# yugabyte/yugabyte-db

Measured on AMD Instinct MI355X. Metric: scanned_rows_per_s, higher is better.
Workload: dtype int64; 1 GPU; 1 tablet, 100M rows, 4KB SST blocks, three_shared_parts, packed-row V2, 3 int64 predicates + SUM(int64); rows=100000000, tablets=1, block_size=4096

## Files before the change

### yugabyte-db_amd/csrc/fast_sim_main.cc

```cpp
#include <cstdio>
#include <cstdlib>
#include <cstring>
#include <vector>

#include "../../include/yb_gpu_scan.h"

extern "C" int ybg_sim_scan(const ybg_scan_spec_t*, const uint8_t*,
                            const uint64_t*, uint64_t, ybg_scan_result_t*);
extern "C" int ybg_sim_scan_fast(const ybg_scan_spec_t*, const uint8_t*,
                                 const uint64_t*, uint64_t,
                                 ybg_scan_result_t*, uint64_t*);

namespace {

constexpr uint64_t kSlack = 48;
constexpr uint64_t kMvccBase = 1600000000000000ull;

ybg_schema_t make_schema(int ncols) {
  ybg_schema_t s;
  memset(&s, 0, sizeof(s));
  s.has_hash = 1;
  s.num_hash_cols = 1;
  s.key_types[0] = YBG_KT_INT64;
  s.num_value_cols = ncols;
  for (int i = 0; i < ncols; ++i) s.value_cols[i] = {10 + i, YBG_T_INT64, 1};
  return s;
}

struct Query {
  int num_preds;
  ybg_pred_t preds[3];
  ybg_agg_t aggs[2];
  uint64_t read, local;
};

bool same(const ybg_scan_result_t& a, const ybg_scan_result_t& b) {
  bool ok = a.rows_scanned == b.rows_scanned &&
            a.rows_matched == b.rows_matched &&
            a.entries_seen == b.entries_seen &&
            a.restart_ht_len == b.restart_ht_len &&
            !memcmp(a.restart_ht, b.restart_ht, a.restart_ht_len);
  for (int g = 0; g < 2 && ok; ++g)
    ok = a.aggs[g].is_null == b.aggs[g].is_null &&
         (a.aggs[g].is_null || a.aggs[g].value_i64 == b.aggs[g].value_i64);
  return ok;
}

int check(const char* what, const ybg_schema_t& schema, const uint8_t* data,
          const uint64_t* offsets, uint64_t n_blocks, uint64_t total,
          const Query& q) {
  uint8_t* exact = (uint8_t*)malloc(total + kSlack);
  memcpy(exact, data, total);
  memset(exact + total, 0, kSlack);
  ybg_scan_spec_t spec;
  memset(&spec, 0, sizeof(spec));
  spec.schema = schema;
  spec.kv_format = YBG_ENC_THREE_SHARED_PARTS;
  ybg_read_time_init(&spec.read_time, q.read << 12, q.local << 12,
                     q.local << 12);
  spec.num_preds = q.num_preds;
  for (int i = 0; i < q.num_preds; ++i) spec.preds[i] = q.preds[i];
  spec.num_aggs = 2;
  spec.aggs[0] = q.aggs[0];
  spec.aggs[1] = q.aggs[1];
  int bad = 0;
  uint64_t nf_max = 0;
  for (const char* ivb : {"1", "2", "4"}) {
    setenv("YBG_IVB", ivb, 1);
    ybg_scan_result_t want;
    spec.expect_versions = 0;
    bad |= ybg_sim_scan(&spec, exact, offsets, n_blocks, &want);
    for (const char* plan : {"1", "0"}) {
      setenv("YBG_PLAN", plan, 1);
      for (int fuse = 0; fuse < 2; ++fuse) {
        spec.expect_versions = fuse;
        ybg_scan_result_t got;
        uint64_t nf = 0;
        int rc = ybg_sim_scan_fast(&spec, exact, offsets, n_blocks, &got, &nf);
        if (rc || !same(got, want)) {
          printf("  %s ivb=%s plan=%s fuse=%d: rc=%d MISMATCH\n", what, ivb,
                 plan, fuse, rc);
          bad = 1;
        }
        if (nf > nf_max) nf_max = nf;
      }
    }
    if (!strcmp(ivb, "1"))
      printf("%s: blocks=%llu bytes=%llu scanned=%llu matched=%llu "
             "fallbacks<=%llu %s\n",
             what, (unsigned long long)n_blocks, (unsigned long long)total,
             (unsigned long long)want.rows_scanned,
             (unsigned long long)want.rows_matched,
             (unsigned long long)nf_max, bad ? "MISMATCH" : "ok");
  }
  free(exact);
  return bad;
}

int check_generated(const char* tag, int ncols, uint64_t rows, int versions,
                    const Query& q) {
  ybg_schema_t schema = make_schema(ncols);
  ybg_gen_params_t p;
  memset(&p, 0, sizeof(p));
  p.rows = rows;
  p.seed = 42;
  p.packed_version = 2;
  p.kv_format = YBG_ENC_THREE_SHARED_PARTS;
  p.block_size = 4096;
  p.restart_interval = 16;
  p.versions = versions;
  p.ht_base_micros = kMvccBase;
  p.ht_step_micros = versions > 1 ? 1000000 : 1000;
  p.nthreads = 1;
  uint8_t* data;
  uint64_t* offsets;
  uint64_t n_blocks, total, n_entries;
  if (ybg_generate(&schema, &p, &data, &offsets, &n_blocks, &total,
                   &n_entries))
    return 1;
  char what[64];
  snprintf(what, sizeof(what), "%s rows=%llu", tag, (unsigned long long)rows);
  int bad = check(what, schema, data, offsets, n_blocks, total, q);
  ybg_free(data);
  ybg_free(offsets);
  return bad;
}

int check_built(const char* tag, int kind, uint64_t rows, const Query& q) {
  const int ncols = (kind == 1 || kind >= 4) ? 4 : 1;
  ybg_schema_t schema = make_schema(ncols);
  ybg_builder_t* b = ybg_builder_create(&schema, YBG_ENC_THREE_SHARED_PARTS,
                                        4096, kind >= 2 ? 1 : 16);
  uint64_t seq = 1ull << 50;
  int rc = 0;
  for (uint64_t r = 0; r < rows && !rc; ++r) {
    ybg_key_t k;
    memset(&k, 0, sizeof(k));
    k.hash = (uint16_t)(r / 64);
    k.datums[0] = r;
    ybg_rowvals_t v;
    memset(&v, 0, sizeof(v));
    uint64_t ht = 2000;
    if (kind == 0) {
      v.datums[0] = r * 11 + 1;
      if (r % 7 == 3) {
        rc = ybg_builder_add_row_tombstone(b, &k, 3000ull << 12, 0, seq++);
        continue;
      }
      if (r % 5 == 0)
        rc = ybg_builder_add_row_tombstone(b, &k, 3000ull << 12, 0, seq++);
    } else if (kind == 1) {
      for (int c = 0; c < 4; ++c) v.datums[c] = r * 3 + c;
      if (r % 37 == 20)
        rc = ybg_builder_add_column_update(b, &k, 2, 3000ull << 12, 0, seq++,
                                           r + 5, nullptr, 0, 0);
    } else if (kind >= 4) {
      for (int c = 0; c < 4; ++c) v.datums[c] = r * 8 + c;
      ht = 1000;
      if (kind == 5 && r + 1 == rows) {
        rc = ybg_builder_add_row_tombstone(b, &k, ht << 12, 0, seq++);
        continue;
      }
    } else {
      v.datums[0] = kind == 2 ? (uint64_t)INT64_MAX - r * 3 : r;
      ht = (kind == 3 && r == 137) ? 3000 : 1000;
    }
    if (!rc)
      rc = ybg_builder_add_packed_row(b, &k, ht << 12, 0, seq++, 2, &v);
  }
  const uint8_t* data;
  const uint64_t* offsets;
  uint64_t n_blocks, total, n_entries;
  if (rc || ybg_builder_finish(b, &data, &offsets, &n_blocks, &total,
                               &n_entries))
    return 1;
  char what[64];
  snprintf(what, sizeof(what), "%s rows=%llu", tag, (unsigned long long)rows);
  int bad = check(what, schema, data, offsets, n_blocks, total, q);
  ybg_builder_destroy(b);
  return bad;
}

}

int main() {
  const uint64_t kRead = 1700000000000000ull;
  Query headline = {3,
                    {{0, 0, YBG_PRED_GT, 1ull << 39, nullptr, 0},
                     {0, 1, YBG_PRED_LT, 3ull << 38, nullptr, 0},
                     {0, 2, YBG_PRED_GE, 1ull << 36, nullptr, 0}},
                    {{YBG_AGG_SUM_INT64, 3}, {YBG_AGG_COUNT_STAR, 0}},
                    kRead, kRead};
  Query one_col = {1,
                   {{0, 0, YBG_PRED_GT, 1ull << 39, nullptr, 0}},
                   {{YBG_AGG_COUNT_STAR, 0}, {YBG_AGG_SUM_INT64, 0}},
                   kRead, kRead};
  Query count_sum0 = {0, {}, {{YBG_AGG_COUNT_STAR, 0}, {YBG_AGG_SUM_INT64, 0}},
                      5000, 5000};
  Query mvcc = count_sum0, below = count_sum0, restart = count_sum0;
  mvcc.read = mvcc.local = kMvccBase + 2500000;
  below.read = below.local = kMvccBase - 1;
  restart.read = 2000;
  restart.local = 4000;
  Query tomb = count_sum0, upd = headline;
  tomb.num_preds = 1;
  tomb.preds[0] = {0, 0, YBG_PRED_GT, 50, nullptr, 0};
  upd.num_preds = 1;
  upd.preds[0] = {0, 0, YBG_PRED_GE, 30, nullptr, 0};
  upd.read = upd.local = 5000;

  int bad = 0;
  for (uint64_t n : {1, 2, 15, 16, 17, 31, 32, 33, 90, 91, 92, 93, 94, 182,
                     183, 184, 185, 186, 2000, 6000}) {
    bad |= check_generated("four-column", 4, n, 1, headline);
    bad |= check_generated("one-column", 1, n, 1, one_col);
  }
  bad |= check_generated("four-column", 4, 200000, 1, headline);
  for (uint64_t n : {1, 17, 33, 93, 2000}) {
    bad |= check_generated("mvcc", 4, n, 5, mvcc);
    bad |= check_generated("mvcc-below", 4, n, 5, below);
  }
  bad |= check_built("tombstones", 0, 700, tomb);
  bad |= check_built("column-update", 1, 600, upd);
  for (uint64_t n : {1, 63, 64, 65, 255, 256, 257})
    bad |= check_built("epilogue", 2, n, count_sum0);
  bad |= check_built("restart-one", 3, 200, restart);
  Query wide = headline;
  wide.num_preds = 3;
  wide.preds[0] = {0, 0, YBG_PRED_GE, 8, nullptr, 0};
  wide.preds[1] = {0, 1, YBG_PRED_LT, 8 * 90, nullptr, 0};
  wide.preds[2] = {0, 2, YBG_PRED_GE, 18, nullptr, 0};
  wide.read = wide.local = 5000;
  for (uint64_t n : {1, 2, 93, 94, 200}) {
    bad |= check_built("last-restart-sum-last-column", 4, n, wide);
    bad |= check_built("last-restart-tombstone", 5, n, wide);
  }
  printf(bad ? "FAILED\n" : "all ok\n");
  return bad;
}
```

### yugabyte-db_amd/csrc/scan_device.h

```cpp
#pragma once
#include <cstdint>
#include <cstdlib>
#include <cstring>

#include "../../include/yb_gpu_scan.h"

#ifndef YBG_DEV_QUAL
#define YBG_DEV_QUAL __device__ __forceinline__
#endif
#define DEV YBG_DEV_QUAL

#ifdef YBG_HOST_SIM
static inline double __longlong_as_double(long long v) {
  double d;
  memcpy(&d, &v, 8);
  return d;
}
static inline long long __double_as_longlong(double d) {
  long long v;
  memcpy(&v, &d, 8);
  return v;
}
static inline float __uint_as_float(unsigned v) {
  float f;
// ... 2189 lines not shown
      d = rc.emit_datums[c];
      if (((rc.emit_str >> c) & 1) && !ec->varlen) {
        d = 0;
      } else if ((rc.emit_str >> c) & 1) {
        uint32_t sl = rc.emit_lens[c];
        unsigned long long off = atomicAdd(ec->varlen_counter, sl);
        if (off + sl > ec->varlen_cap) {
          atomicAdd(ec->overflow, 1ull);
          d = 0;
        } else {
          const uint8_t* src = (const uint8_t*)(uintptr_t)d;
          for (uint32_t i = 0; i < sl; ++i) ec->varlen[off + i] = src[i];
          d = ((uint64_t)sl << 40) | off;
        }
      }
    }
    ec->datums[slot * nc + c] = d;
  }
  ec->null_masks[slot] = rc.emit_null;
  ec->hashes[slot] =
      sp.has_hash ? (uint16_t)(((uint16_t)rk[1] << 8) | rk[2]) : 0;
}


DEV void combine_datum(int op, uint64_t* val, uint64_t* cnt, uint64_t v) {
  switch (op) {
    case YBG_AGG_COUNT_STAR:
    case YBG_AGG_COUNT:
      *val += 1;
      break;
    case YBG_AGG_SUM_INT64:
      *val += v;
      break;
    case YBG_AGG_SUM_DOUBLE: {
      double cur = __longlong_as_double((long long)*val) +
                   __longlong_as_double((long long)v);
      *val = (uint64_t)__double_as_longlong(cur);
      break;
    }
    case YBG_AGG_MIN_INT64:
      if (*cnt == 0 || (int64_t)v < (int64_t)*val) *val = v;
      break;
    case YBG_AGG_MAX_INT64:
      if (*cnt == 0 || (int64_t)v > (int64_t)*val) *val = v;
      break;
    case YBG_AGG_MIN_DOUBLE: {
      double dd = __longlong_as_double((long long)v);
      if (*cnt == 0 || dd < __longlong_as_double((long long)*val))
        *val = (uint64_t)__double_as_longlong(dd);
      break;
    }
    case YBG_AGG_MAX_DOUBLE: {
      double dd = __longlong_as_double((long long)v);
      if (*cnt == 0 || dd > __longlong_as_double((long long)*val))
        *val = (uint64_t)__double_as_longlong(dd);
      break;
    }
  }
  *cnt += 1;
}

DEV bool pred_cmp_fast(const PredC& pr, uint64_t datum) {
  const int dtype = (int)(pr.opdt >> 8);
  int cmp;
  if (YBG_LIKELY(dtype != YBG_T_DOUBLE && dtype != YBG_T_FLOAT)) {
    int64_t a = (int64_t)datum, b = (int64_t)pr.datum;
    cmp = a < b ? -1 : (a > b ? 1 : 0);
  } else if (dtype == YBG_T_DOUBLE) {
    double a = __longlong_as_double((long long)datum);
    double b = __longlong_as_double((long long)pr.datum);
    cmp = a < b ? -1 : (a > b ? 1 : 0);
  } else {
    float a = __uint_as_float((uint32_t)datum);
    float b = __uint_as_float((uint32_t)pr.datum);
    cmp = a < b ? -1 : (a > b ? 1 : 0);
  }
  switch (pr.opdt & 0xff) {
    case YBG_PRED_GT: return cmp > 0;
    case YBG_PRED_GE: return cmp >= 0;
    case YBG_PRED_LT: return cmp < 0;
    case YBG_PRED_LE: return cmp <= 0;
    case YBG_PRED_EQ: return cmp == 0;
    default: return cmp != 0;
  }
}

inline bool fast_eligible(const DevSpec& d) {
  if (d.fmt != YBG_ENC_THREE_SHARED_PARTS) return false;
  if (!d.fixed_rk_len || d.need_rowkey || d.group_col >= 0) return false;
  if (!d.v2_fixed_len || d.num_value_cols <= 0) return false;
  if (d.num_value_cols > 8) return false;
  if (d.num_aggs > 2) return false;
  for (int i = 0; i < d.num_preds; ++i) {
    if (d.preds[i].is_key_col) return false;
    if (d.preds[i].op > YBG_PRED_NE) return false;
  }
  return true;
}

constexpr int kPlanMaxCols = 8;
constexpr int kPlanAggs = 2;
constexpr int kPlanGroupSlots = 4;
constexpr int kPlanShapeP1 = 16;
constexpr int kPlanShapeP1S1 = 17;
constexpr int kPlanShapeP2 = 18;
constexpr int plan_np(int nc) {
  return nc == kPlanShapeP2 ? 2 : (nc >= kPlanShapeP1 ? 1 : 0);
}
constexpr int plan_ns(int nc) {
  return nc < kPlanShapeP1 ? nc : (nc == kPlanShapeP1S1 ? 1 : 0);
}

struct FastPlan {
  int64_t lo[kPlanMaxCols], hi[kPlanMaxCols];
  uint8_t off[kPlanMaxCols];
  uint32_t n_rng;
  uint32_t agg_off[kPlanAggs];
  uint32_t agg_mask[kPlanAggs];
  uint32_t agg_one[kPlanAggs];
  uint32_t agg_on[kPlanAggs];
  uint32_t shape;
  uint32_t agg_sel[kPlanAggs][kPlanGroupSlots];
  uint32_t rkb, v2_fixed_len, track_restart;
  HtLim reg_lim;
};

inline bool build_fast_plan(const DevSpec& d, FastPlan* pl) {
  memset(pl, 0, sizeof(*pl));
  for (int k = 0; k < kPlanMaxCols; ++k) {
    pl->lo[k] = INT64_MIN;
    pl->hi[k] = INT64_MAX;
  }
  if (!fast_eligible(d) || d.num_aggs > kPlanAggs) return false;
  auto wide = [&](int c) {
    return c >= 0 && c < d.num_value_cols && d.cols[c].v2_fixed == 8;
  };
  int rng_of[YBG_MAX_COLS];
  for (int c = 0; c < YBG_MAX_COLS; ++c) rng_of[c] = -1;
  for (int i = 0; i < d.num_preds; ++i) {
    const DevPred& pr = d.preds[i];
    if (pr.op < YBG_PRED_GT || pr.op > YBG_PRED_EQ) return false;
    if (!wide(pr.col)) return false;
    const int dt = d.cols[pr.col].dtype;
    if (dt != YBG_T_INT64 && dt != YBG_T_UINT64) return false;
    if (rng_of[pr.col] < 0) {
      rng_of[pr.col] = (int)pl->n_rng;
      pl->off[pl->n_rng++] = d.v2_off[pr.col];
    }
    const int k = rng_of[pr.col];
    const int64_t c = (int64_t)pr.datum;
    int64_t lo = INT64_MIN, hi = INT64_MAX;
    bool empty = false;
    switch (pr.op) {
      case YBG_PRED_GT:
        if (c == INT64_MAX) empty = true; else lo = c + 1;
        break;
      case YBG_PRED_GE: lo = c; break;
      case YBG_PRED_LT:
        if (c == INT64_MIN) empty = true; else hi = c - 1;
        break;
      case YBG_PRED_LE: hi = c; break;
      default: lo = hi = c; break;
    }
    if (lo > pl->lo[k]) pl->lo[k] = lo;
    if (hi < pl->hi[k]) pl->hi[k] = hi;
    if (empty || pl->lo[k] > pl->hi[k]) {
      pl->lo[k] = INT64_MAX;
      pl->hi[k] = INT64_MIN;
    }
  }
  for (int g = 0; g < d.num_aggs; ++g) {
    const int op = d.aggs[g].op;
    pl->agg_on[g] = 1;
    if (op == YBG_AGG_COUNT_STAR) {
      pl->agg_one[g] = 1;
    } else if (op == YBG_AGG_COUNT) {
      if (d.aggs[g].col < 0 || d.aggs[g].col >= d.num_value_cols)
        return false;
      pl->agg_one[g] = 1;
    } else if (op == YBG_AGG_SUM_INT64) {
      if (!wide(d.aggs[g].col)) return false;
      pl->agg_off[g] = d.v2_off[d.aggs[g].col];
      pl->agg_mask[g] = ~0u;
    } else {
      return false;
    }
  }
  pl->rkb = d.fixed_rk_len;
  pl->v2_fixed_len = d.v2_fixed_len;
  pl->track_restart = (uint32_t)d.track_restart;
  pl->reg_lim = d.reg_lim;
  pl->shape = pl->n_rng <= 4 ? pl->n_rng : (uint32_t)kPlanMaxCols;
  struct Live {
    uint32_t off;
    int64_t lo, hi;
  };
  Live lv[kPlanMaxCols + kPlanAggs];
  int n = 0;
  for (uint32_t k = 0; k < pl->n_rng; ++k)
    lv[n++] = Live{pl->off[k], pl->lo[k], pl->hi[k]};
  for (int g = 0; g < d.num_aggs; ++g) {
    if (!pl->agg_mask[g]) continue;
    bool have = false;
    for (int i = 0; i < n; ++i) have |= lv[i].off == pl->agg_off[g];
    if (!have) lv[n++] = Live{pl->agg_off[g], INT64_MIN, INT64_MAX};
  }
  for (int i = 1; i < n; ++i)
    for (int j = i; j > 0 && lv[j].off < lv[j - 1].off; --j) {
      const Live t = lv[j];
      lv[j] = lv[j - 1];
      lv[j - 1] = t;
    }
  Live pr[kPlanMaxCols + kPlanAggs], sg[kPlanMaxCols + kPlanAggs];
  int np = 0, ns = 0;
  for (int i = 0; i < n;) {
    if (i + 1 < n && lv[i + 1].off == lv[i].off + 8) {
      pr[2 * np] = lv[i];
      pr[2 * np + 1] = lv[i + 1];
      ++np;
      i += 2;
    } else {
      sg[ns++] = lv[i++];
    }
  }
  const int shape = (np == 1 && ns == 0)   ? kPlanShapeP1
                    : (np == 1 && ns == 1) ? kPlanShapeP1S1
                    : (np == 2 && ns == 0) ? kPlanShapeP2
                                           : -1;
  if (shape >= 0) {
    for (int k = 0; k < kPlanMaxCols; ++k) {
      pl->lo[k] = INT64_MIN;
      pl->hi[k] = INT64_MAX;
      pl->off[k] = 0;
    }
    Live slot[kPlanGroupSlots];
    for (int k = 0; k < 2 * np; ++k) slot[k] = pr[k];
    for (int k = 0; k < ns; ++k) slot[2 * np + k] = sg[k];
    for (int k = 0; k < np; ++k) pl->off[k] = (uint8_t)pr[2 * k].off;
    for (int k = 0; k < ns; ++k) pl->off[np + k] = (uint8_t)sg[k].off;
    for (int k = 0; k < 2 * np + ns; ++k) {
      pl->lo[k] = slot[k].lo;
      pl->hi[k] = slot[k].hi;
      for (int g = 0; g < d.num_aggs; ++g)
        if (pl->agg_mask[g] && pl->agg_off[g] == slot[k].off)
          pl->agg_sel[g][k] = ~0u;
    }
    pl->shape = (uint32_t)shape;
  }
  return true;
}

inline int fast_plan_nr(const FastPlan& pl) { return (int)pl.shape; }

inline bool fast_plan_enabled() {
  const char* e = getenv("YBG_PLAN");
  return !e || atoi(e) != 0;
}

template <int N, class OffT>
DEV void plan_load_cols(const OffT* off, const uint8_t* value, uint64_t* uv) {
#pragma unroll
  for (int k = 0; k < N; ++k) uv[k] = load_u64_direct_g(value + off[k]);
}
template <int NP, int NS>
DEV void plan_load_groups(const uint8_t* off, const uint8_t* value,
                          uint64_t* uv) {
#pragma unroll
  for (int k = 0; k < NP; ++k) {
    const U64x2 v = load_u128_direct_g(value + off[k]);
    uv[2 * k] = v.lo;
    uv[2 * k + 1] = v.hi;
  }
#pragma unroll
  for (int k = 0; k < NS; ++k)
    uv[2 * NP + k] = load_u64_direct_g(value + off[NP + k]);
}

#ifndef YBG_FABORT
#define YBG_FABORT(n) return 0
#endif
#ifndef YBG_CENSUS_REC
#define YBG_CENSUS_REC(kind, sp, ns1, ns2, l1, l2) ((void)0)
#endif

template <int NA, int NC, bool FUSE = false, bool PLAN = false>
DEV int scan_batch_fast(const DevSpec& sp, const uint8_t* data,
                        const uint64_t* block_offsets, const Interval* ivs,
                        uint64_t n_ivs, uint64_t j_lo, uint64_t j_hi,
                        uint8_t* key, uint64_t* rmin,
                        uint32_t* entries, uint32_t* scanned,
                        uint32_t* matched, uint64_t* agg_val,
                        uint64_t* agg_cnt, HeadOut<NA>* ho,
                        bool* walked_next_out,
                        const FastPlan* pl = nullptr) {
  static_assert(!PLAN || (NA == kPlanAggs &&
                          (NC <= kPlanMaxCols ||
                           (NC >= kPlanShapeP1 && NC <= kPlanShapeP2))),
                "plan shape");
  Interval iv = ivs[j_lo];
  const uint8_t* blk = data + block_offsets[iv.block];
  const uint8_t* p = blk + iv.start;
  const uint8_t* limit = blk + iv.end;
  uint64_t cur_iv = j_lo;
  Rdr rdr;
  rdr.init(p);
  bool at_restart = true;

#pragma unroll
  for (int g = 0; g < NA; ++g) { ho->val[g] = 0; ho->cnt[g] = 0; }
  ho->scanned = 0;
  ho->matched = 0;

  uint32_t e_b = 0, s_b = 0, m_b = 0;
  uint64_t av_b[NA], ac_b[NA];
#pragma unroll
  for (int g = 0; g < NA; ++g) { av_b[g] = 0; ac_b[g] = 0; }

  uint32_t key_len = 0;
  uint64_t thi = 0, tlo = 0;
  bool row_open = false, in_head = true, walked = false;
  bool base_seen = false, found = false;
  uint32_t pred_pass = 0, agg_null = 0xffffffffu;
  bool row_pass = true;
  uint64_t agg_datum[NA];
#pragma unroll
  for (int g = 0; g < NA; ++g) agg_datum[g] = 0;
  const uint32_t rkb = PLAN ? pl->rkb : sp.fixed_rk_len;
  const HtLim& reg_lim = PLAN ? pl->reg_lim : sp.reg_lim;
  EntryRef er;
  auto acc_row = [&](uint32_t* sc, uint32_t* mt, uint64_t* val,
                     uint64_t* cnt) {
    *sc += 1;
    if constexpr (PLAN) {
      if (row_pass) {
        *mt += 1;
#pragma unroll
        for (int g = 0; g < NA; ++g) {
          const uint32_t m = pl->agg_mask[g];
          const uint64_t d = ((uint64_t)((uint32_t)(agg_datum[g] >> 32) & m)
                              << 32) |
                             ((uint32_t)agg_datum[g] & m);
          val[g] += d + pl->agg_one[g];
          cnt[g] += pl->agg_on[g];
        }
      }
    } else {
      if ((pred_pass & sp.value_pred_mask) == sp.value_pred_mask) {
        *mt += 1;
#pragma unroll
        for (int g = 0; g < NA; ++g) {
          if (g >= sp.num_aggs) continue;
          bool nul = (sp.agg_op[g] != YBG_AGG_COUNT_STAR) &&
                     ((agg_null >> g) & 1);
          if (!nul)
            combine_datum(sp.agg_op[g], &val[g], &cnt[g], agg_datum[g]);
        }
      }
    }
  };

  for (;;) {
    if (p >= limit) {
      if (cur_iv + 1 >= n_ivs) break;
      Interval nx = ivs[cur_iv + 1];
      cur_iv += 1;
      at_restart = true;
      const uint8_t* nblk = data + block_offsets[nx.block];
      const uint8_t* np = nblk + nx.start;
      limit = nblk + nx.end;
      blk = nblk;
      YBG_CENSUS_REC(0, 0, 0, 0, 0, 0);
      if (np != p) {
        p = np;
        rdr.init(p);
      }
      continue;
    }
    bool kchg;
    const uint8_t* q = nullptr;
    if (YBG_UNLIKELY(at_restart)) {
      at_restart = false;
      if (limit - p < 3) YBG_FABORT(1);
      uint64_t w = load_u64_direct_g(p);
      uint32_t b0 = (uint32_t)(w & 0xff);
      uint64_t e1;
      uint32_t e1len;
      if (!(b0 & 0x80)) {
        e1 = b0;
        e1len = 1;
      } else {
        uint32_t b1 = (uint32_t)((w >> 8) & 0xff);
        if (b1 & 0x80) YBG_FABORT(2);
        e1 = (b0 & 0x7f) | ((uint64_t)b1 << 7);
        e1len = 2;
      }
      uint32_t value_size = (uint32_t)(e1 >> 2);
      if (e1 & 1) YBG_FABORT(3);
      uint32_t e2 = (uint32_t)((w >> (8 * e1len)) & 0xff);
      if (e2 & 1) YBG_FABORT(4);
      uint32_t ns1 = e2 >> 1;
      static_assert(kFastKeyCap % 16 == 0, "chunk copy fills whole chunks");
      if (ns1 < 24 || ns1 > kFastKeyCap - 8) YBG_FABORT(5);
      uint32_t hl = e1len + 1;
      if ((uint64_t)(limit - p) < (uint64_t)hl + ns1 + value_size) YBG_FABORT(6);
      const uint8_t* kp2 = p + hl;
      const U64x2 c0 = load_u128_direct_g(kp2);
      const U64x2 c1 = load_u128_direct_g(kp2 + 16);
      U64x2 c2{0, 0};
      if (ns1 > 32) c2 = load_u128_direct_g(kp2 + 32);
      thi = __builtin_bswap64(load_u64_direct_g(kp2 + ns1 - 24));
      tlo = __builtin_bswap64(load_u64_direct_g(kp2 + ns1 - 16));
      key_len = ns1;
      er.value = kp2 + ns1;
      er.value_len = value_size;
      er.shared = 0;
      q = er.value + value_size;
      rdr.seek(er.value);
      auto word_chg = [&](uint32_t i, uint64_t nw) -> bool {
        if (i >= rkb) return false;
        const uint64_t m =
            rkb - i >= 8 ? ~0ull : (1ull << (8 * (rkb - i))) - 1;
        return ((lds_load_u64(&key[i]) ^ nw) & m) != 0;
      };
      kchg = !row_open;
      if (row_open) {
        kchg |= word_chg(0, c0.lo);
        kchg |= word_chg(8, c0.hi);
        kchg |= word_chg(16, c1.lo);
        kchg |= word_chg(24, c1.hi);
        kchg |= word_chg(32, c2.lo);
        kchg |= word_chg(40, c2.hi);
      }
      lds_store_u128(&key[0], c0);
      lds_store_u128(&key[16], c1);
      if (ns1 > 32) lds_store_u128(&key[32], c2);
      for (uint32_t i = 48; i < ns1; i += 16) {
        const U64x2 c = load_u128_direct_g(kp2 + i);
        if (row_open) {
          kchg |= word_chg(i, c.lo);
          kchg |= word_chg(i + 8, c.hi);
        }
        lds_store_u128(&key[i], c);
      }
      YBG_CENSUS_REC(1, 0, ns1, 0, 0, 0);
    } else {
      if (limit - p < 8) YBG_FABORT(7);
      rdr.align8();
      uint64_t w = rdr.peek8();
      uint32_t b0 = (uint32_t)(w & 0xff);
      uint64_t e1;
      uint32_t e1len;
      if (!(b0 & 0x80)) {
        e1 = b0;
        e1len = 1;
      } else {
        uint32_t b1 = (uint32_t)((w >> 8) & 0xff);
        if (b1 & 0x80) YBG_FABORT(8);
        e1 = (b0 & 0x7f) | ((uint64_t)b1 << 7);
        e1len = 2;
      }
      const uint32_t value_size = (uint32_t)(e1 >> 2);
      const uint64_t inc = (e1 & 2) << 7;
      uint32_t ns1, ns2, hl, sp;
      int form;
      uint64_t w2 = rdr.peek8_at(8);
      auto hdr_byte = [&](uint32_t j) -> uint32_t {
        return (uint32_t)((j < 8 ? (w >> (8 * j)) : (w2 >> (8 * (j - 8)))) &
                          0xff);
      };
      if (e1 & 1) {
        sp = hdr_byte(e1len);
        if (sp & 0x80) YBG_FABORT(9);
        ns1 = 1;
        ns2 = 1;
        hl = e1len + 1;
        form = 2;
      } else {
        uint32_t e2 = hdr_byte(e1len);
        if ((e2 & 3) == 1) {
          if (e2 & 4) YBG_FABORT(10);
          ns1 = (e2 >> 3) & 7;
          ns2 = (e2 >> 6) & 3;
          sp = hdr_byte(e1len + 1);
          if (sp & 0x80) YBG_FABORT(11);
          hl = e1len + 2;
          form = 3;
        } else if ((e2 & 7) == 7 && !(e2 & 40)) {
          uint32_t o = e1len + 1;
          ns1 = hdr_byte(o);
          if (ns1 & 0x80) YBG_FABORT(12);
          ++o;
          ns2 = 0;
          if (e2 & 16) {
            ns2 = hdr_byte(o);
            if (ns2 & 0x80) YBG_FABORT(13);
            ++o;
          }
          sp = hdr_byte(o);
          if (sp & 0x80) YBG_FABORT(14);
          hl = o + 1;
          form = 4;
        } else {
          YBG_FABORT(15);
        }
      }
      const uint32_t nb = hl + ns1 + ns2;
      if (nb > 24 || ns1 > 16 || ns2 > 8) YBG_FABORT(16);
      const uint64_t prev_len = key_len;
      const uint64_t prev_except = (uint64_t)sp + ns1 + ns2 + 8;
      if (prev_len < prev_except ||
          (uint64_t)(limit - p) < (uint64_t)nb + value_size)
        YBG_FABORT(17);
      const uint32_t ukey = (uint32_t)prev_len - 8;
      const uint32_t ns2s = (uint32_t)(prev_len - ns2 - 8);
      kchg = sp < rkb || !row_open;
      {
        rdr.align8();
        w = rdr.peek8();
        w2 = rdr.peek8_at(8);
        uint64_t w3 = rdr.peek8_at(16);
        auto body_byte = [&](uint32_t j) -> uint8_t {
          uint64_t src = j < 8 ? w : (j < 16 ? w2 : w3);
          return (uint8_t)(src >> (8 * (j & 7)));
        };
        uint32_t lds_n = sp < rkb ? (rkb - sp < ns1 ? rkb - sp : ns1) : 0;
        uint32_t lds2 = ns2s < rkb ? (rkb - ns2s < ns2 ? rkb - ns2s : ns2)
                                   : 0;
        YBG_CENSUS_REC(form, sp, ns1, ns2, FUSE ? ns1 : lds_n,
                       FUSE ? ns2 : lds2);
        if constexpr (FUSE) {
          (void)lds_n;
          (void)lds2;
          for (uint32_t i = 0; i < ns1; ++i) {
            uint8_t b = body_byte(hl + i);
            key[sp + i] = b;
            tail_patch(&thi, &tlo, ukey, sp + i, b);
          }
          for (uint32_t i = 0; i < ns2; ++i) {
            uint8_t b = body_byte(hl + ns1 + i);
            key[ns2s + i] = b;
            tail_patch(&thi, &tlo, ukey, ns2s + i, b);
          }
        } else {
          for (uint32_t i = 0; i < lds_n; ++i)
            key[sp + i] = body_byte(hl + i);
          for (uint32_t i = 0; i < lds2; ++i)
            key[ns2s + i] = body_byte(hl + ns1 + i);
          for (uint32_t i = 0; i < ns1; ++i)
            tail_patch(&thi, &tlo, ukey, sp + i, body_byte(hl + i));
          for (uint32_t i = 0; i < ns2; ++i)
            tail_patch(&thi, &tlo, ukey, ns2s + i, body_byte(hl + ns1 + i));
        }
      }
      (void)inc;
      (void)form;
      rdr.consume(nb);
      er.value = rdr.pos();
      er.value_len = value_size;
      q = er.value + value_size;
    }
    const uint32_t ukey_len = key_len - 8;
    if (ukey_len < rkb + 2 || ukey_len < 16) YBG_FABORT(19);
    const uint32_t ht_sz = (uint32_t)tlo & 0x1f;
    if (ht_sz == 0 || ht_sz >= 16) YBG_FABORT(20);
    const uint32_t mb = ht_sz + 1;
    uint32_t marker;
    if (mb <= 8) marker = (uint32_t)(tlo >> (8 * (mb - 1))) & 0xff;
    else marker = (uint32_t)(thi >> (8 * (mb - 9))) & 0xff;
    if (marker != kHybridTimeByte) YBG_FABORT(21);
    if (ukey_len != rkb + ht_sz + 1) YBG_FABORT(22);
    uint64_t ht_hi, ht_lo;
    {
      uint32_t s = 8 * (16 - ht_sz);
      if (s == 0) { ht_hi = thi; ht_lo = tlo; }
      else if (s < 64) {
        ht_hi = (thi << s) | (tlo >> (64 - s));
        ht_lo = tlo << s;
      } else {
        ht_hi = tlo << (s - 64);
        ht_lo = 0;
      }
    }
    if (kchg) {
      if (row_open) {
        if (found) {
          if (in_head) acc_row(&ho->scanned, &ho->matched, ho->val, ho->cnt);
          else acc_row(&s_b, &m_b, av_b, ac_b);
        }
        in_head = false;
        row_open = false;
        if (cur_iv >= j_hi) break;
      }
      row_open = true;
      base_seen = false;
      found = false;
      pred_pass = 0;
      agg_null = 0xffffffffu;
      row_pass = true;
    }
    e_b += (cur_iv < j_hi);
    walked |= (cur_iv == j_hi);
    const uint32_t vb0 =
        er.value_len ? (uint32_t)(rdr.peek8() & 0xff) : 0u;
    if (YBG_UNLIKELY(vb0 == kHybridTimeByte)) YBG_FABORT(23);
    const bool visible =
        u128_slice_cmp(ht_hi, ht_lo, ht_sz, reg_lim.hi, reg_lim.lo,
                       reg_lim.len) >= 0;
    if (visible) {
      if (YBG_UNLIKELY(PLAN ? pl->track_restart : sp.track_restart)) {
        if (u128_slice_cmp(ht_hi, ht_lo, ht_sz, sp.read.hi, sp.read.lo,
                           sp.read.len) < 0) {
          uint64_t* rr = rmin;
          if (rr[2] == 0 || u128_slice_cmp(ht_hi, ht_lo, ht_sz, rr[0],
                                           rr[1], (uint32_t)rr[2]) < 0) {
            rr[0] = ht_hi;
            rr[1] = ht_lo;
            rr[2] = ht_sz;
          }
        }
      }
      if (!base_seen) {
        base_seen = true;
        if (YBG_LIKELY(er.value_len ==
                           (PLAN ? pl->v2_fixed_len : sp.v2_fixed_len) &&
                       vb0 == kPackedV2B &&
                       (rdr.peek8() & 0xff8000u) == 0)) {
          const uint8_t* value = rdr.pos();
          rdr.seek(value + er.value_len);
          if constexpr (PLAN) {
            constexpr int NP = plan_np(NC), NS = plan_ns(NC);
            constexpr int NSL = 2 * NP + NS;
            uint64_t uv[NSL > 0 ? NSL : 1];
            if constexpr (NP > 0) {
              plan_load_groups<NP, NS>(pl->off, value, uv);
            } else {
              plan_load_cols<NC>(pl->off, value, uv);
#pragma unroll
              for (int g = 0; g < NA; ++g)
                if (pl->agg_mask[g])
                  agg_datum[g] = load_u64_direct_g(value + pl->agg_off[g]);
            }
#pragma unroll
            for (int k = 0; k < NSL; ++k) {
              const int64_t v = (int64_t)uv[k];
              row_pass &= (v >= pl->lo[k]) & (v <= pl->hi[k]);
            }
            if constexpr (NP > 0) {
#pragma unroll
              for (int g = 0; g < NA; ++g) {
                uint32_t dl = 0, dh = 0;
#pragma unroll
                for (int k = 0; k < NSL; ++k) {
                  const uint32_t m = pl->agg_sel[g][k];
                  dl |= (uint32_t)uv[k] & m;
                  dh |= (uint32_t)(uv[k] >> 32) & m;
                }
                agg_datum[g] = ((uint64_t)dh << 32) | dl;
              }
            }
          } else {
            const uintptr_t a = (uintptr_t)value;
            GPtr<uint64_t> qw =
                gptr<uint64_t>((const void*)(a & ~(uintptr_t)7));
            const uint32_t abase = (uint32_t)(a & 7);
            uint64_t uv[NC];
#pragma unroll
            for (int i = 0; i < NC; ++i) {
              const uint32_t ob = abase + sp.v2_off[i];
              const uint32_t wi = ob >> 3, shb = (ob & 7) * 8;
              const uint64_t w0 = qw[wi], w1 = qw[wi + 1];
              uv[i] = shb ? (w0 >> shb) | (w1 << (64 - shb)) : w0;
            }
#pragma unroll
            for (int i = 0; i < NC; ++i) {
              const uint32_t act = sp.col_act[i];
              uint64_t u = uv[i];
              const uint32_t dt = (act >> kActDtShift) & kActDtM;
              switch ((act >> kActV2Shift) & kActV2M) {
                case 1:
                  u = (dt == YBG_T_INT8) ? (uint64_t)(int64_t)(int8_t)u
                                         : (u & 0xff);
                  break;
                case 2:
                  u = (dt == YBG_T_INT16) ? (uint64_t)(int64_t)(int16_t)u
                                          : (u & 0xffff);
                  break;
                case 4:
                  u = (dt == YBG_T_INT32) ? (uint64_t)(int64_t)(int32_t)u
                                          : (u & 0xffffffffull);
                  break;
                default:
                  break;
              }
              uint32_t pm = act & kActPredM;
              while (pm) {
                int pi = __builtin_ctz(pm);
                pm &= pm - 1;
                bool pass = pred_cmp_fast(sp.predc[pi], u);
                pred_pass =
                    (pred_pass & ~(1u << pi)) | ((uint32_t)pass << pi);
              }
              uint32_t am = (act >> kActAggShift) & kActAggM;
              if (am) {
#pragma unroll
                for (int g = 0; g < NA; ++g) {
                  if (am & (1u << g)) {
                    agg_datum[g] = u;
                    agg_null &= ~(1u << g);
                  }
                }
              }
            }
          }
          found = true;
          p = q;
          continue;
        } else if (er.value_len == 1 && vb0 == kTombB) {
        } else {
          YBG_FABORT(24);
        }
      }
    }
    rdr.seek(q);
    p = q;
  }
  if (row_open && found) {
    if (in_head) acc_row(&ho->scanned, &ho->matched, ho->val, ho->cnt);
    else acc_row(&s_b, &m_b, av_b, ac_b);
  }
  *entries += e_b;
  *scanned += s_b;
  *matched += m_b;
#pragma unroll
  for (int g = 0; g < NA; ++g) {
    if (g < sp.num_aggs)
      combine1(sp.agg_op[g], &agg_val[g], &agg_cnt[g], av_b[g], ac_b[g]);
  }
  *walked_next_out = walked;
  return 1;
}

template <int NA, bool EMIT, bool GROUP>
DEV void finalize_row(const DevSpec& sp, const RowCtxT<NA>& rc,
                      const uint8_t* rkp, uint32_t rk_len,
                      const uint8_t* aux, bool in_head, uint64_t j,
                      uint32_t* scanned, uint32_t* matched,
                      uint64_t* agg_val, uint64_t* agg_cnt, HeadOut<NA>* ho,
                      EmitCtx* ec, uint64_t row_sort_key, const GroupCtx* gc,
                      GroupHead* gh_out) {
  if (!rc.found || !in_bounds(sp, rkp, rk_len, aux)) return;
  bool hit = (rc.pred_pass & sp.value_pred_mask) == sp.value_pred_mask &&
             eval_key_preds(sp, rkp, rk_len, aux);
  if (in_head) {
    ho->scanned += 1;
    if (hit) {
      ho->matched += 1;
      acc_row(sp, rc, ho->val, ho->cnt);
    }
  } else {
    *scanned += 1;
    if (hit) {
      *matched += 1;
      acc_row(sp, rc, agg_val, agg_cnt);
    }
  }
  if (!hit) return;
  if (EMIT && (!in_head || ec->head_consumed[j] == 0))
    emit_row(sp, ec, rc, rkp, rk_len, row_sort_key);
  if (GROUP) {
    if (!in_head) {
      group_accum(sp, *gc, rc);
    } else {
      gh_out->grp_datum = rc.grp_datum;
      gh_out->grp_len = rc.grp_len;
      gh_out->grp_null = rc.grp_null ? 1u : 0u;
      gh_out->agg_null = rc.agg_null;
#pragma unroll
      for (int g = 0; g < NA; ++g) gh_out->agg_datum[g] = rc.agg_datum[g];
      gh_out->hit = 1;
    }
  }
}

template <int NA, bool EMIT = false, bool GROUP = false>
DEV bool scan_one_interval(const DevSpec& sp, const uint8_t* data,
                           const uint64_t* block_offsets, const Interval* ivs,
                           uint64_t n_ivs, uint64_t j, uint64_t j_hi,
                           const uint8_t* aux, uint8_t* key,
                           uint8_t* rk_save, uint64_t* bht,
                           uint32_t* entries,
                           uint32_t* scanned, uint32_t* matched,
                           uint64_t* agg_val, uint64_t* agg_cnt,
                           HeadOut<NA>* ho, bool* walked_next_out,
                           uint32_t* iv_flags,
                           EmitCtx* ec = nullptr,
                           uint64_t* emit_datums = nullptr,
                           uint32_t* emit_lens = nullptr,
                           const GroupCtx* gc = nullptr,
                           GroupHead* gh_out = nullptr) {
  Interval iv = ivs[j];
  const uint8_t* blk = data + block_offsets[iv.block];
  const uint8_t* p = blk + iv.start;
  const uint8_t* limit = blk + iv.end;
  uint64_t cur_iv = j;
  bool crossed = false;
  Rdr rdr;
  rdr.init(p);

#pragma unroll
  for (int g = 0; g < NA; ++g) { ho->val[g] = 0; ho->cnt[g] = 0; }
  ho->scanned = 0;
  ho->matched = 0;
  bool walked_next = false;
  bool fail = false;

  uint32_t key_len = 0;
  uint64_t reg_last8 = 0;
  uint64_t thi = 0, tlo = 0;
  bool tail_ok = false;
  uint32_t rk_len = 0;
  bool row_open = false;
  bool in_head = true;
  RowCtxT<NA> rc;
  rc.bht = bht;
  rc.emit_datums = EMIT ? emit_datums : nullptr;
  rc.emit_lens = EMIT ? emit_lens : nullptr;
  row_reset(&rc, sp);
  EntryRef er;
  uint64_t row_sort_key = 0;
  const uint32_t rkb =
      (sp.fixed_rk_len && !sp.need_rowkey) ? sp.fixed_rk_len : 0;

  for (;;) {
    if (p >= limit) {
      if (cur_iv + 1 >= n_ivs) break;
      Interval nx = ivs[cur_iv + 1];
      cur_iv += 1;
      crossed = true;
      const uint8_t* nblk = data + block_offsets[nx.block];
      const uint8_t* np = nblk + nx.start;
      limit = nblk + nx.end;
      if (np != p) {
        blk = nblk;
        p = np;
        rdr.init(p);
      } else {
        blk = nblk;
      }
      continue;
    }
    bool kchg = false;
    const uint8_t* q = decode_entry(sp.fmt, &rdr, limit, key, &key_len,
                                    &reg_last8, rkb, &kchg, &er, &thi, &tlo,
                                    &tail_ok);
    if (!q || key_len < 10) { fail = true; break; }
    uint32_t ukey_len = key_len - 8;
    uint32_t ht_sz;
    uint64_t ht_hi, ht_lo;
    if (YBG_LIKELY(ukey_len >= 16)) {
      if (!tail_ok) {
        tail_from_lds(key, ukey_len, &thi, &tlo);
        tail_ok = true;
      }
      ht_sz = (uint32_t)tlo & 0x1f;
      uint32_t mb = ht_sz + 1;
      uint32_t marker;
      if (mb <= 8) marker = (uint32_t)(tlo >> (8 * (mb - 1))) & 0xff;
      else if (mb <= 16) marker = (uint32_t)(thi >> (8 * (mb - 9))) & 0xff;
      else marker = key[ukey_len - mb];
      if (ht_sz == 0 || ukey_len < ht_sz + 2 ||
          marker != kHybridTimeByte) { fail = true; break; }
      uint32_t s = 8 * (16 - ht_sz);
      if (s == 0) { ht_hi = thi; ht_lo = tlo; }
      else if (s < 64) {
        ht_hi = (thi << s) | (tlo >> (64 - s));
        ht_lo = tlo << s;
      } else {
        ht_hi = tlo << (s - 64);
        ht_lo = 0;
      }
    } else {
      ht_sz = key[ukey_len - 1] & 0x1f;
      if (ht_sz == 0 || ukey_len < ht_sz + 2 ||
          key[ukey_len - ht_sz - 1] != kHybridTimeByte) { fail = true; break; }
      slice_u128(key + ukey_len - ht_sz, ht_sz, &ht_hi, &ht_lo);
    }
    uint32_t prefix_len = ukey_len - ht_sz - 1;
    uint32_t rk;
    if (sp.fixed_rk_len) {
      rk = sp.fixed_rk_len;
      if (rk > prefix_len) { fail = true; break; }
    } else {
      rk = dockey_len(sp, key, prefix_len);
      if (!rk || rk > prefix_len) { fail = true; break; }
    }

    bool row_change;
    if (rkb) {
      row_change = !row_open || kchg;
    } else {
      row_change = !row_open || (rk != rk_len);
      if (!row_change && er.shared < rk) {
        for (uint32_t i = er.shared; i < rk; ++i) {
          if (key[i] != rk_save[i]) { row_change = true; break; }
        }
      }
    }
    if (row_change) {
      if (row_open) {
        finalize_row<NA, EMIT, GROUP>(
            sp, rc, (rkb && !EMIT) ? key : rk_save, rk_len, aux, in_head, j,
            scanned, matched, agg_val, agg_cnt, ho, ec, row_sort_key, gc,
            gh_out);
        in_head = false;
        row_open = false;
        if (cur_iv >= j_hi) break;
      }
      if (!rkb || EMIT) {
        for (uint32_t i = 0; i < rk; ++i) rk_save[i] = key[i];
      }
      rk_len = rk;
      row_open = true;
      if (EMIT)
        row_sort_key = ((uint64_t)cur_iv << 16) | (uint64_t)(p - blk);
      row_reset(&rc, sp);
    }
    if (iv_flags && crossed && !row_change) iv_flags[cur_iv] = 1;
    crossed = false;
    *entries += (cur_iv < j_hi);
    walked_next |= (cur_iv == j_hi);
    if (!process_entry(sp, data, aux, key, key_len, er.value, er.value_len,
                       rk_len, &rc, &rdr, ht_sz, ht_hi, ht_lo)) {
      fail = true;
      break;
    }
    rdr.seek(q);
    p = q;
  }
  if (!fail && row_open)
    finalize_row<NA, EMIT, GROUP>(
        sp, rc, (rkb && !EMIT) ? key : rk_save, rk_len, aux, in_head, j,
        scanned, matched, agg_val, agg_cnt, ho, ec, row_sort_key, gc, gh_out);
  *walked_next_out = walked_next;
  return !fail;
}


inline uint32_t unpack_restart_ht(uint64_t hi, uint64_t lo, uint64_t len,
                                  uint8_t* out) {
  uint32_t n = (uint32_t)len;
  if (n > YBG_MAX_HT) n = YBG_MAX_HT;
  for (uint32_t i = 0; i < n; ++i)
    out[i] = (uint8_t)(
        (i < 8 ? hi >> (56 - 8 * i) : lo >> (56 - 8 * (i - 8))) & 0xff);
  return n;
}

inline void build_dev_spec(const ybg_scan_spec_t* spec, DevSpec* dp,
                           unsigned char* aux, uint32_t* aux_len,
                           uint32_t aux_cap) {
  DevSpec& d = *dp;
  memset(&d, 0, sizeof(d));
  const ybg_schema_t& sc = spec->schema;
  d.has_hash = sc.has_hash;
  d.num_hash_cols = sc.num_hash_cols;
  d.num_range_cols = sc.num_range_cols;
  for (int i = 0; i < YBG_MAX_KEYCOLS; ++i) d.key_types[i] = sc.key_types[i];
  d.num_value_cols = sc.num_value_cols;
  d.fuse_hint = spec->expect_versions != 0;
  int nvar = 0, off_after = 0;
  for (int i = 0; i < sc.num_value_cols; ++i) {
    DevCol& c = d.cols[i];
    c.id = sc.value_cols[i].column_id;
    c.dtype = sc.value_cols[i].dtype;
    bool varlen =
        sc.value_cols[i].nullable || sc.value_cols[i].dtype == YBG_T_STRING;
    c.v1_varlen = varlen;
    c.v1_nvb = nvar;
    c.v1_off = off_after;
    int v1sz;
    switch (sc.value_cols[i].dtype) {
      case YBG_T_BOOL: v1sz = 1; break;
      case YBG_T_INT8: case YBG_T_INT16: case YBG_T_INT32:
      case YBG_T_UINT32: case YBG_T_FLOAT: v1sz = 5; break;
      default: v1sz = 9; break;
    }
    if (varlen) { ++nvar; off_after = 0; }
    else off_after += v1sz;
    switch (sc.value_cols[i].dtype) {
      case YBG_T_BOOL: case YBG_T_INT8: c.v2_fixed = 1; break;
      case YBG_T_INT16: c.v2_fixed = 2; break;
      case YBG_T_INT32: case YBG_T_UINT32: case YBG_T_FLOAT:
        c.v2_fixed = 4; break;
      case YBG_T_STRING: c.v2_fixed = 0; break;
      default: c.v2_fixed = 8; break;
    }
  }
  d.v1_varlen_count = nvar;
  d.fmt = spec->kv_format;
  auto htlim = [](const uint8_t* b, int32_t len, HtLim* o) {
    uint64_t hi = 0, lo = 0;
    for (int i = 0; i < len && i < 16; ++i) {
      uint64_t v = b[i];
      if (i < 8) hi |= v << (56 - 8 * i);
      else lo |= v << (56 - 8 * (i - 8));
    }
    o->hi = hi;
    o->lo = lo;
    o->len = (uint32_t)len;
  };
  htlim(spec->read_time.read, spec->read_time.read_len, &d.read);
  htlim(spec->read_time.local_limit, spec->read_time.local_limit_len,
        &d.local_lim);
  htlim(spec->read_time.global_limit, spec->read_time.global_limit_len,
        &d.global_lim);
  {
    int rl = spec->read_time.read_len, ll = spec->read_time.local_limit_len;
    int n = rl < ll ? rl : ll;
    int cmp = memcmp(spec->read_time.local_limit, spec->read_time.read, n);
    bool local_smaller = cmp < 0 || (cmp == 0 && ll < rl);
    d.reg_lim = local_smaller ? d.local_lim : d.read;
    int gl = spec->read_time.global_limit_len;
    int n2 = gl < rl ? gl : rl;
    int cmp2 = memcmp(spec->read_time.global_limit, spec->read_time.read,
                      n2);
    bool global_beyond = cmp2 < 0 || (cmp2 == 0 && gl < rl);
// ... 120 lines not shown
```

Before: 31.60 billion rows/s.

## Software-pipeline entry header and value loads in plan-based block walker

In the plan path the walker now prefetches the next entry's 16-byte header with a direct 128-bit load while it processes the current entry. When the key changes, it also issues the packed-row column loads early, before the MVCC visibility checks. Together these replace the sequential reader's align/peek/seek chain and are meant to hide global-memory latency across entries. The cost is more live registers, possibly lower occupancy, and speculative column loads for rows that turn out not to be visible. New tests cover version chains with tombstones and a two-key schema.

```diff
diff --git a/yugabyte-db_amd/csrc/fast_sim_main.cc b/yugabyte-db_amd/csrc/fast_sim_main.cc
--- a/yugabyte-db_amd/csrc/fast_sim_main.cc
+++ b/yugabyte-db_amd/csrc/fast_sim_main.cc
@@ -16,12 +16,13 @@
 constexpr uint64_t kSlack = 48;
 constexpr uint64_t kMvccBase = 1600000000000000ull;
 
-ybg_schema_t make_schema(int ncols) {
+ybg_schema_t make_schema(int ncols, int nkeys = 1) {
   ybg_schema_t s;
   memset(&s, 0, sizeof(s));
   s.has_hash = 1;
   s.num_hash_cols = 1;
-  s.key_types[0] = YBG_KT_INT64;
+  s.num_range_cols = nkeys - 1;
+  for (int i = 0; i < nkeys; ++i) s.key_types[i] = YBG_KT_INT64;
   s.num_value_cols = ncols;
   for (int i = 0; i < ncols; ++i) s.value_cols[i] = {10 + i, YBG_T_INT64, 1};
   return s;
@@ -128,9 +129,10 @@
 
 int check_built(const char* tag, int kind, uint64_t rows, const Query& q) {
   const int ncols = (kind == 1 || kind >= 4) ? 4 : 1;
-  ybg_schema_t schema = make_schema(ncols);
-  ybg_builder_t* b = ybg_builder_create(&schema, YBG_ENC_THREE_SHARED_PARTS,
-                                        4096, kind >= 2 ? 1 : 16);
+  ybg_schema_t schema = make_schema(ncols, kind == 7 ? 2 : 1);
+  ybg_builder_t* b = ybg_builder_create(
+      &schema, YBG_ENC_THREE_SHARED_PARTS, 4096,
+      (kind >= 2 && kind <= 5) ? 1 : 16);
   uint64_t seq = 1ull << 50;
   int rc = 0;
   for (uint64_t r = 0; r < rows && !rc; ++r) {
@@ -154,6 +156,26 @@
       if (r % 37 == 20)
         rc = ybg_builder_add_column_update(b, &k, 2, 3000ull << 12, 0, seq++,
                                            r + 5, nullptr, 0, 0);
+    } else if (kind == 6) {
+      if (r + 1 == rows) {
+        rc = ybg_builder_add_row_tombstone(b, &k, 2000ull << 12, 0, seq++);
+        continue;
+      }
+      if (r % 5 == 1)
+        rc = ybg_builder_add_row_tombstone(b, &k, 9000ull << 12, 0, seq++);
+      if (!rc && r % 3 == 0)
+        rc = ybg_builder_add_row_tombstone(b, &k, 4000ull << 12, 0, seq++);
+      for (uint64_t ver = 3; ver >= 1 && !rc; --ver) {
+        for (int c = 0; c < 4; ++c) v.datums[c] = r * 8 + c + ver * 1000;
+        if (ver > 1)
+          rc = ybg_builder_add_packed_row(b, &k, (ver * 1000) << 12, 0, seq++,
+                                          2, &v);
+      }
+      ht = 1000;
+    } else if (kind == 7) {
+      k.datums[1] = r << 40;
+      for (int c = 0; c < 4; ++c) v.datums[c] = r * 8 + c;
+      ht = kMvccBase + r * 1000;
     } else if (kind >= 4) {
       for (int c = 0; c < 4; ++c) v.datums[c] = r * 8 + c;
       ht = 1000;
@@ -235,6 +257,17 @@
     bad |= check_built("last-restart-sum-last-column", 4, n, wide);
     bad |= check_built("last-restart-tombstone", 5, n, wide);
   }
+  Query chains = wide, keys2 = wide;
+  chains.preds[1] = {0, 1, YBG_PRED_LT, 1ull << 40, nullptr, 0};
+  keys2.preds[1] = chains.preds[1];
+  keys2.read = keys2.local = kMvccBase + 1000000000ull;
+  for (uint64_t n : {2, 17, 33, 200}) {
+    for (uint64_t rd : {1500, 2500, 3500, 5000}) {
+      chains.read = chains.local = rd;
+      bad |= check_built("chains-tombstone-last", 6, n, chains);
+    }
+    bad |= check_built("two-keys-long-headers", 7, n, keys2);
+  }
   printf(bad ? "FAILED\n" : "all ok\n");
   return bad;
 }
diff --git a/yugabyte-db_amd/csrc/scan_device.h b/yugabyte-db_amd/csrc/scan_device.h
--- a/yugabyte-db_amd/csrc/scan_device.h
+++ b/yugabyte-db_amd/csrc/scan_device.h
@@ -2515,8 +2515,11 @@
   const uint8_t* p = blk + iv.start;
   const uint8_t* limit = blk + iv.end;
   uint64_t cur_iv = j_lo;
+  constexpr bool PIPE = PLAN && !(FUSE && NC == 0);
   Rdr rdr;
-  rdr.init(p);
+  U64x2 wa{0, 0};
+  if constexpr (PIPE) wa = load_u128_direct_g(p);
+  else rdr.init(p);
   bool at_restart = true;
 
 #pragma unroll
@@ -2585,16 +2588,42 @@
       YBG_CENSUS_REC(0, 0, 0, 0, 0, 0);
       if (np != p) {
         p = np;
-        rdr.init(p);
+        if constexpr (PIPE) wa = load_u128_direct_g(p);
+        else rdr.init(p);
       }
       continue;
     }
     bool kchg;
     const uint8_t* q = nullptr;
+    uint32_t vw = 0;
+    constexpr int NSL =
+        !PLAN ? 0 : plan_np(NC) > 0 ? 2 * plan_np(NC) + plan_ns(NC) : NC;
+    uint64_t uv[NSL > 0 ? NSL : 1];
+    uint64_t ad[NA];
+    bool cols_early = false;
+    (void)uv;
+    (void)ad;
+    auto load_cols = [&](const uint8_t* value) {
+      if constexpr (PLAN) {
+        constexpr int NP = plan_np(NC), NS = plan_ns(NC);
+        if constexpr (NP > 0) {
+          plan_load_groups<NP, NS>(pl->off, value, uv);
+        } else {
+          plan_load_cols<NC>(pl->off, value, uv);
+#pragma unroll
+          for (int g = 0; g < NA; ++g) {
+            ad[g] = 0;
+            if (pl->agg_mask[g])
+              ad[g] = load_u64_direct_g(value + pl->agg_off[g]);
+          }
+        }
+      }
+    };
+    U64x2 na{0, 0};
     if (YBG_UNLIKELY(at_restart)) {
       at_restart = false;
       if (limit - p < 3) YBG_FABORT(1);
-      uint64_t w = load_u64_direct_g(p);
+      uint64_t w = PIPE ? wa.lo : load_u64_direct_g(p);
       uint32_t b0 = (uint32_t)(w & 0xff);
       uint64_t e1;
       uint32_t e1len;
@@ -2628,7 +2657,13 @@
       er.value_len = value_size;
       er.shared = 0;
       q = er.value + value_size;
-      rdr.seek(er.value);
+      uint64_t vq = 0;
+      if constexpr (PIPE) {
+        vq = load_u64_direct_g(er.value);
+        na = load_u128_direct_g(q);
+      } else {
+        rdr.seek(er.value);
+      }
       auto word_chg = [&](uint32_t i, uint64_t nw) -> bool {
         if (i >= rkb) return false;
         const uint64_t m =
@@ -2655,11 +2690,20 @@
         }
         lds_store_u128(&key[i], c);
       }
+      if constexpr (PIPE) vw = (uint32_t)vq;
+      else vw = (uint32_t)rdr.peek8();
       YBG_CENSUS_REC(1, 0, ns1, 0, 0, 0);
     } else {
       if (limit - p < 8) YBG_FABORT(7);
-      rdr.align8();
-      uint64_t w = rdr.peek8();
+      uint64_t w, w2, w3 = 0, w4 = 0;
+      if constexpr (PIPE) {
+        w = wa.lo;
+        w2 = wa.hi;
+      } else {
+        rdr.align8();
+        w = rdr.peek8();
+        w2 = rdr.peek8_at(8);
+      }
       uint32_t b0 = (uint32_t)(w & 0xff);
       uint64_t e1;
       uint32_t e1len;
@@ -2676,7 +2720,6 @@
       const uint64_t inc = (e1 & 2) << 7;
       uint32_t ns1, ns2, hl, sp;
       int form;
-      uint64_t w2 = rdr.peek8_at(8);
       auto hdr_byte = [&](uint32_t j) -> uint32_t {
         return (uint32_t)((j < 8 ? (w >> (8 * j)) : (w2 >> (8 * (j - 8)))) &
                           0xff);
@@ -2727,11 +2770,31 @@
       const uint32_t ukey = (uint32_t)prev_len - 8;
       const uint32_t ns2s = (uint32_t)(prev_len - ns2 - 8);
       kchg = sp < rkb || !row_open;
+      if constexpr (PIPE) {
+        if (YBG_UNLIKELY(nb > 13)) {
+          const U64x2 wb = load_u128_direct_g(p + 16);
+          w3 = wb.lo;
+          w4 = wb.hi;
+        }
+      }
+      const uint8_t* const value = p + nb;
+      q = value + value_size;
+      if constexpr (PIPE) {
+        if constexpr (!FUSE) {
+          if (value_size == pl->v2_fixed_len && (kchg || !base_seen)) {
+            load_cols(value);
+            cols_early = true;
+          }
+        }
+        na = load_u128_direct_g(q);
+      }
       {
-        rdr.align8();
-        w = rdr.peek8();
-        w2 = rdr.peek8_at(8);
-        uint64_t w3 = rdr.peek8_at(16);
+        if constexpr (!PIPE) {
+          rdr.align8();
+          w = rdr.peek8();
+          w2 = rdr.peek8_at(8);
+          w3 = rdr.peek8_at(16);
+        }
         auto body_byte = [&](uint32_t j) -> uint8_t {
           uint64_t src = j < 8 ? w : (j < 16 ? w2 : w3);
           return (uint8_t)(src >> (8 * (j & 7)));
@@ -2767,10 +2830,17 @@
       }
       (void)inc;
       (void)form;
-      rdr.consume(nb);
-      er.value = rdr.pos();
+      if constexpr (PIPE) {
+        const uint32_t wi = nb >> 3, sh = 8 * (nb & 7);
+        const uint64_t lo = wi == 0 ? w : wi == 1 ? w2 : wi == 2 ? w3 : w4;
+        const uint64_t hi = wi == 0 ? w2 : wi == 1 ? w3 : w4;
+        vw = (uint32_t)(sh ? (lo >> sh) | (hi << (64 - sh)) : lo);
+      } else {
+        rdr.consume(nb);
+        vw = (uint32_t)rdr.peek8();
+      }
+      er.value = value;
       er.value_len = value_size;
-      q = er.value + value_size;
     }
     const uint32_t ukey_len = key_len - 8;
     if (ukey_len < rkb + 2 || ukey_len < 16) YBG_FABORT(19);
@@ -2813,8 +2883,7 @@
     }
     e_b += (cur_iv < j_hi);
     walked |= (cur_iv == j_hi);
-    const uint32_t vb0 =
-        er.value_len ? (uint32_t)(rdr.peek8() & 0xff) : 0u;
+    const uint32_t vb0 = er.value_len ? (vw & 0xff) : 0u;
     if (YBG_UNLIKELY(vb0 == kHybridTimeByte)) YBG_FABORT(23);
     const bool visible =
         u128_slice_cmp(ht_hi, ht_lo, ht_sz, reg_lim.hi, reg_lim.lo,
@@ -2837,21 +2906,16 @@
         if (YBG_LIKELY(er.value_len ==
                            (PLAN ? pl->v2_fixed_len : sp.v2_fixed_len) &&
                        vb0 == kPackedV2B &&
-                       (rdr.peek8() & 0xff8000u) == 0)) {
-          const uint8_t* value = rdr.pos();
-          rdr.seek(value + er.value_len);
+                       (vw & 0xff8000u) == 0)) {
+          const uint8_t* value = er.value;
+          if constexpr (!PIPE) rdr.seek(q);
           if constexpr (PLAN) {
-            constexpr int NP = plan_np(NC), NS = plan_ns(NC);
-            constexpr int NSL = 2 * NP + NS;
-            uint64_t uv[NSL > 0 ? NSL : 1];
-            if constexpr (NP > 0) {
-              plan_load_groups<NP, NS>(pl->off, value, uv);
-            } else {
-              plan_load_cols<NC>(pl->off, value, uv);
+            constexpr int NP = plan_np(NC);
+            if (!cols_early) load_cols(value);
+            if constexpr (NP == 0) {
 #pragma unroll
               for (int g = 0; g < NA; ++g)
-                if (pl->agg_mask[g])
-                  agg_datum[g] = load_u64_direct_g(value + pl->agg_off[g]);
+                if (pl->agg_mask[g]) agg_datum[g] = ad[g];
             }
 #pragma unroll
             for (int k = 0; k < NSL; ++k) {
@@ -2926,6 +2990,7 @@
             }
           }
           found = true;
+          if constexpr (PIPE) wa = na;
           p = q;
           continue;
         } else if (er.value_len == 1 && vb0 == kTombB) {
@@ -2934,7 +2999,8 @@
         }
       }
     }
-    rdr.seek(q);
+    if constexpr (PIPE) wa = na;
+    else rdr.seek(q);
     p = q;
   }
   if (row_open && found) {
```

Result: faster. 35.56 billion rows/s (median of 6 runs) (+12.5%).
